# rofuyu/exp-trmf-nips16

Hardware: AMD Instinct MI355X
Metric: als_iterations_per_sec (higher is better)
Workload: dtype f32

## Files before the change

### exp-trmf-nips16_amd/csrc/gram_kernels.hpp

```cpp
#pragma once

#include <type_traits>
#include <utility>

#include "common.hpp"

namespace trmf {

template <typename T> struct Mfma16;
template <> struct Mfma16<float> {
    typedef float acc_t __attribute__((ext_vector_type(4)));
    static __device__ __forceinline__ acc_t mma(float a, float b, acc_t c) {
        return __builtin_amdgcn_mfma_f32_16x16x4f32(a, b, c, 0, 0, 0);
    }
    static __device__ __forceinline__ int row(int lane, int r) { return 4 * (lane >> 4) + r; }
};
template <> struct Mfma16<double> {
    typedef double acc_t __attribute__((ext_vector_type(4)));
    static __device__ __forceinline__ acc_t mma(double a, double b, acc_t c) {
        return __builtin_amdgcn_mfma_f64_16x16x4f64(a, b, c, 0, 0, 0);
    }
    static __device__ __forceinline__ int row(int lane, int r) { return (lane >> 4) + 4 * r; }
};

// ... 486 lines not shown

template <int NT, int KMAX, bool RHS_IN>
__device__ __forceinline__ void quad_factor_solve(quad_f4 (&a4)[NT][KMAX / 4], float (&bz)[NT], float (&x)[NT], int c) {
    constexpr int NR = KMAX / 4;
    float dinv[NT];
#pragma unroll
    for (int q = 0; q < NT; q++) dinv[q] = 0;
    static_for<KMAX>([&](auto J) {
        constexpr int j = decltype(J)::value, qj = j >> 4, cj = j & 15, Rj = j >> 2, ij = j & 3;
        {
            const float inv = __builtin_amdgcn_rsqf(row_bcast<cj>(a4[qj][Rj][ij]));
            float u[NT], nu[NT];
#pragma unroll
            for (int q = qj; q < NT; q++) {
                u[q] = a4[q][Rj][ij] * inv;
                if (q == qj && c <= cj) u[q] = 0;
                a4[q][Rj][ij] = u[q];
                nu[q] = -u[q];
            }
            if constexpr (!RHS_IN) {
                const float zj = row_bcast<cj>(bz[qj]) * inv;
#pragma unroll
                for (int q = qj; q < NT; q++) bz[q] = fmaf(-u[q], zj, bz[q]);
                if (c == cj) bz[qj] = zj;
            }
            if (c == cj) dinv[qj] = inv;
            static_for<NR>([&](auto Rx) {
                constexpr int R = decltype(Rx)::value, qs = (4 * R) >> 4;
                if constexpr (4 * R + 3 > j) {
#pragma unroll
                    for (int q = qs; q < NT; q++) a4[q][R] = __builtin_amdgcn_mfma_f32_4x4x1f32(nu[qs], u[q], a4[q][R], 2, R & 3, 0);
                }
            });
            __builtin_amdgcn_sched_barrier(0);
        }
    });
#pragma unroll
    for (int q = 0; q < NT; q++) x[q] = 0;
    if constexpr (RHS_IN) {
        if (c == 15) x[NT - 1] = -1.0f;
#pragma unroll
        for (int q = 0; q < NT; q++) bz[q] = 0;
    }
    static_for<KMAX>([&](auto Jr) {
        constexpr int j = KMAX - 1 - decltype(Jr)::value, qj = j >> 4, cj = j & 15, Rj = j >> 2, ij = j & 3;
        {
            float part = 0;
#pragma unroll
            for (int q = qj; q < NT; q++) part = fmaf(a4[q][Rj][ij], x[q], part);
            const float sum = row16_allsum_dpp(part);
            const float xv = (bz[qj] - sum) * dinv[qj];
            if (c == cj) x[qj] = xv;
        }
    });
}

struct QuadStream {
    uint32_t pr[5];
    uint32_t step;
    uint32_t long_m1;
    __device__ __forceinline__ uint32_t row_ptr_at(int i) const {
        return i == 0 ? pr[0] : i == 1 ? pr[1] : i == 2 ? pr[2] : i == 3 ? pr[3] : pr[4];
    }
    __device__ __forceinline__ bool skips(int r) const { return row_ptr_at(r + 1) - row_ptr_at(r) - 1u >= long_m1; }
    __device__ __forceinline__ GramDesc first() const {
        GramDesc d{0, 0, -1};
        for (int r = 0; r < 4; r++)
            if (!skips(r)) { d = GramDesc{row_ptr_at(r), row_ptr_at(r + 1), r}; break; }
        return d;
    }
    __device__ __forceinline__ void operator()(GramDesc &d) const {
        if (d.row < 0) return;
        d.e0 += step;
        if (d.e0 < d.end) return;
        int r = d.row + 1;
        while (r < 4 && skips(r)) r++;
        if (r < 4) d = GramDesc{row_ptr_at(r), row_ptr_at(r + 1), r};
        else d = GramDesc{0, 0, -1};
    }
};

constexpr int kQuadWaves = 3;
constexpr int quad_waves(int NT) { return NT >= 4 ? 2 : kQuadWaves; }
constexpr bool quad_row_end(int NT, int KMAX) { return (NT == 3 && KMAX == 40) || (NT == 4 && KMAX == 56); }
#if !defined(TRMF_UNIT_BODIES)
template <int NT, int KMAX>
__global__ void fsolve_quad_kernel(const uint32_t *__restrict__ ptr,
                                                          const uint32_t *__restrict__ idx,
                                                          const float *__restrict__ val,
                                                          const float *__restrict__ X,
                                                          float *__restrict__ F, uint32_t row_begin,
                                                          uint32_t row_end, int k, float lambda,
                                                          uint32_t zero_row, uint32_t long_m1);
template <int NT, int KMAX>
__global__ void fsolve_quad_long_kernel(SplitRows sp, float *__restrict__ F, int k, float lambda);
#else
template <int NT, int KMAX, bool LONG>
__device__ __forceinline__ void fsolve_quad_body(const uint32_t *__restrict__ ptr,
                                                          const uint32_t *__restrict__ idx,
                                                          const float *__restrict__ val,
                                                          const float *__restrict__ X,
                                                          float *__restrict__ F, uint32_t row_begin,
                                                          uint32_t row_end, int k, float lambda,
                                                          uint32_t zero_row, uint32_t long_m1, const SplitRows &sp) {
    static_assert(sizeof(real) == 4, "quad F-solve is the fp32 path");
    constexpr int KP = kTile * NT;
    constexpr int SLAB = quad_slab_floats<NT>();
    __shared__ __attribute__((aligned(16))) float lds_slab[4][SLAB];
    const int wave = threadIdx.x >> 6, lane = threadIdx.x & 63;
    const int grp = lane >> 4, c = lane & 15;
    const uint32_t row0 = LONG ? sp.begin + (blockIdx.x * 4u + (uint32_t)wave) * 4u : row_begin + (blockIdx.x * 4u + (uint32_t)wave) * 4u;
    if (row0 >= (LONG ? sp.end : row_end)) return;
    float *S = lds_slab[wave];
    typedef float f4 __attribute__((ext_vector_type(4)));

    quad_f4 a4[NT][KMAX / 4];
    float bz[NT];
#pragma unroll
    for (int q = 0; q < NT; q++) {
        bz[q] = 0;
#pragma unroll
        for (int s = 0; s < KMAX; s++) a4[q][s >> 2][s & 3] = (s == kTile * q + c) ? 1.0f : 0.0f;
    }
    bool mine = false;

    QuadStream stream;
    stream.step = 4u * kRingDepth;
    stream.long_m1 = long_m1;
    {
        const uint32_t rr = row0 + (uint32_t)(lane < 5 ? lane : 4);
        const uint32_t lim = LONG ? sp.end : row_end;
        const uint32_t v = (LONG ? sp.first : ptr)[rr < lim ? rr : lim];
#pragma unroll
        for (int i = 0; i < 5; i++) stream.pr[i] = (uint32_t)__builtin_amdgcn_readlane((int)v, i);
    }

    GramState<NT> st;
    st.clear();
    constexpr bool PAD = KMAX <= kTile * NT - 8;
    auto finalize = [&](int sys) {
        if constexpr (!PAD) {
#pragma unroll
            for (int q = 0; q < NT; q++) {
                st.b[q] += __shfl_xor(st.b[q], 16, kWave);
                st.b[q] += __shfl_xor(st.b[q], 32, kWave);
            }
        }
        int t = 0;
#pragma unroll
        for (int ti = 0; ti < NT; ti++)
#pragma unroll
            for (int tj = ti; tj < NT; tj++, t++) {
                f4 v = st.acc[t];
                if (ti == tj) {
#pragma unroll
                    for (int r = 0; r < 4; r++)
                        if (c == 4 * grp + r) v[r] += (kTile * ti + c < k) ? lambda : 1.0f;
                }
                *reinterpret_cast<f4 *>(&S[quad_slab_col_offset<NT>(tj) + c * (kTile * (tj + 1) + 4) + kTile * ti + 4 * grp]) = v;
            }
        __builtin_amdgcn_fence(__ATOMIC_ACQ_REL, "wavefront");
        __builtin_amdgcn_wave_barrier();
        if (grp == sys) {
            mine = true;
#pragma unroll
            for (int q = 0; q < NT; q++) {
                if constexpr (!PAD) bz[q] = st.b[q];
#pragma unroll
                for (int s4 = 0; s4 < KMAX / 4; s4++) {
                    if (4 * s4 <= kTile * q + 15)
                        a4[q][s4] = *reinterpret_cast<const f4 *>(&S[quad_slab_col_offset<NT>(q) + c * (kTile * (q + 1) + 4) + 4 * s4]);
                }
            }
        }
        __builtin_amdgcn_fence(__ATOMIC_ACQ_REL, "wavefront");
        __builtin_amdgcn_wave_barrier();
        st.clear();
    };

    if constexpr (LONG) {
        for (int sys = 0; sys < 4; sys++) {
            if (stream.row_ptr_at(sys + 1) == stream.row_ptr_at(sys)) continue;
            load_row_sum<NT, !PAD>(st, sp, stream.row_ptr_at(sys), lane);
            finalize(sys);
        }
    } else {
        float nowq[NT];
#pragma unroll
        for (int q = 0; q < NT; q++) nowq[q] = 0;
        gram_ring<NT, kRingDepth, true, false, PAD, false, quad_row_end(NT, KMAX)>(st, idx, val, X, zero_row, 4u, lane, nowq, stream.first(), stream,
                                                    finalize);
    }

    float x[NT];
    quad_factor_solve<NT, KMAX, PAD>(a4, bz, x, c);
    if (mine) {
        RealVec<NT> o;
#pragma unroll
        for (int q = 0; q < NT; q++) o.v[q] = (kTile * q + c < k) ? x[q] : 0.0f;
        const uint32_t orow = LONG ? sp.rows[row0 + (uint32_t)grp] : row0 + (uint32_t)grp;
        *reinterpret_cast<RealVec<NT> *>(F + (size_t)orow * KP + NT * c) = o;
    }
}
template <int NT, int KMAX>
__global__ __launch_bounds__(256, quad_waves(NT)) void fsolve_quad_kernel(const uint32_t *__restrict__ ptr,
                                                          const uint32_t *__restrict__ idx,
                                                          const float *__restrict__ val,
                                                          const float *__restrict__ X,
                                                          float *__restrict__ F, uint32_t row_begin,
                                                          uint32_t row_end, int k, float lambda,
                                                          uint32_t zero_row, uint32_t long_m1) {
    fsolve_quad_body<NT, KMAX, false>(ptr, idx, val, X, F, row_begin, row_end, k, lambda, zero_row, long_m1, SplitRows{});
}
template <int NT, int KMAX>
__global__ __launch_bounds__(256, quad_waves(NT) - 1) void fsolve_quad_long_kernel(SplitRows sp, float *__restrict__ F, int k, float lambda) {
    fsolve_quad_body<NT, KMAX, true>(nullptr, nullptr, nullptr, nullptr, F, 0u, 0u, k, lambda, 0u, 0u, sp);
}
#endif

#endif

#if !defined(TRMF_UNIT_BODIES)
template <int NT, bool RHS_PAD, bool PACKED>
__global__ void gram_x_kernel(const uint32_t *__restrict__ ptr,
                                                     const uint32_t *__restrict__ idx,
                                                     const real *__restrict__ val,
                                                     const real *__restrict__ Hf,
                                                     real *__restrict__ G, real *__restrict__ Bv,
                                                     uint32_t row_begin, uint32_t row_end, int k,
                                                     uint32_t zero_row, size_t gs, uint32_t long_thresh, const uint32_t *__restrict__ order);
template <int NT, bool RHS_PAD, bool PACKED>
__global__ void gram_x_long_kernel(SplitRows sp, real *__restrict__ G, real *__restrict__ Bv, int k, size_t gs);
template <int NT, bool RHS_PAD>
__global__ void gram_part_kernel(const uint32_t *__restrict__ idx, const real *__restrict__ val, const real *__restrict__ X,
                                 const uint32_t *__restrict__ items, uint32_t item_begin, uint32_t item_end,
                                 real *__restrict__ slab, uint32_t stride, uint32_t zero_row);
#else
template <int NT, bool RHS_PAD>
__global__ __launch_bounds__(256) void gram_part_kernel(const uint32_t *__restrict__ idx, const real *__restrict__ val,
                                                        const real *__restrict__ X, const uint32_t *__restrict__ items,
                                                        uint32_t item_begin, uint32_t item_end, real *__restrict__ slab,
                                                        uint32_t stride, uint32_t zero_row) {
    typedef typename Mfma16<real>::acc_t acc_t;
    constexpr int NTT = NT * (NT + 1) / 2;
    const int wave = threadIdx.x >> 6, lane = threadIdx.x & 63;
    const uint32_t item = item_begin + blockIdx.x * 4u + (uint32_t)wave;
    if (item >= item_end) return;
    const uint32_t p0 = (uint32_t)__builtin_amdgcn_readfirstlane((int)items[2 * item]);
    const uint32_t p1 = (uint32_t)__builtin_amdgcn_readfirstlane((int)items[2 * item + 1]);
    GramState<NT> st;
    st.clear();
    real nowq[NT];
#pragma unroll
    for (int q = 0; q < NT; q++) nowq[q] = 0;
    if (p1 > p0)
        gram_ring<NT, kRingDepth, true, false, RHS_PAD>(st, idx, val, X, zero_row, 4u, lane, nowq, GramDesc{p0, p1, 0},
                                                        SingleRowStream{4u * kRingDepth}, [](int) {});
    real *p = slab + (size_t)item * stride;
#pragma unroll
    for (int t = 0; t < NTT; t++) *reinterpret_cast<acc_t *>(p + t * 4 * kWave + 4 * lane) = st.acc[t];
    if constexpr (!RHS_PAD) {
#pragma unroll
        for (int q = 0; q < NT; q++) p[NTT * 4 * kWave + q * kWave + lane] = st.b[q];
    }
}

template <int NT, bool RHS_PAD, bool PACKED, bool LONG>
__device__ __forceinline__ void gram_x_body(const uint32_t *__restrict__ ptr,
                                                     const uint32_t *__restrict__ idx,
                                                     const real *__restrict__ val,
                                                     const real *__restrict__ Hf,
                                                     real *__restrict__ G, real *__restrict__ Bv,
                                                     uint32_t row_begin, uint32_t row_end, int k,
                                                     uint32_t zero_row, size_t gs, uint32_t long_thresh, const SplitRows &sp,
                                                     const uint32_t *__restrict__ order) {
    constexpr int KP = kTile * NT;
    const int wave = threadIdx.x >> 6, lane = threadIdx.x & 63;
    const int g = lane >> 4, c = lane & 15;
    GramState<NT> st;
    uint32_t row;
    if constexpr (LONG) {
        const uint32_t li = sp.begin + blockIdx.x * 4u + (uint32_t)wave;
        if (li >= sp.end) return;
        row = (uint32_t)__builtin_amdgcn_readfirstlane((int)sp.rows[li]);
        load_row_sum<NT, !RHS_PAD>(st, sp, (uint32_t)__builtin_amdgcn_readfirstlane((int)sp.first[li]), lane);
    } else {
    row = row_begin + blockIdx.x * (blockDim.x >> 6) + (uint32_t)wave;
    if (row >= row_end) return;
    if (order) row = (uint32_t)__builtin_amdgcn_readfirstlane((int)order[row]);
    const uint32_t p0 = (uint32_t)__builtin_amdgcn_readfirstlane((int)ptr[row]);
    const uint32_t p1 = (uint32_t)__builtin_amdgcn_readfirstlane((int)ptr[row + 1]);
    if (p1 - p0 >= long_thresh) return;

    st.clear();
    real nowq[NT];
#pragma unroll
    for (int q = 0; q < NT; q++) nowq[q] = 0;
    if (p1 > p0)
        gram_ring<NT, kRingDepth, true, false, RHS_PAD>(st, idx, val, Hf, zero_row, 4u, lane, nowq, GramDesc{p0, p1, 0},
// ... 108 lines not shown
```

### exp-trmf-nips16_amd/csrc/kernel_units.hpp

```cpp
#pragma once

#if defined(TRMF_UNIT) || defined(TRMF_SINGLE_UNIT)
#define TRMF_UNIT_BODIES 1
#endif
#if !defined(TRMF_UNIT) || TRMF_UNIT == 1
#include "gram_kernels.hpp"
#endif
#if !defined(TRMF_UNIT) || TRMF_UNIT == 2
#include "cg_kernels.hpp"
#endif
#if defined(TRMF_UNIT) && TRMF_UNIT == 4
#include "cg_kernels.hpp"
#include "gram_kernels.hpp"
#include "full_kernels.hpp"
#endif
#if !defined(TRMF_UNIT) || TRMF_UNIT == 5
#include "heldout_kernels.hpp"
#endif
#if !defined(TRMF_UNIT) || TRMF_UNIT == 6
#include "forecast_kernels.hpp"
#endif
#if !defined(TRMF_UNIT) || TRMF_UNIT == 7
#include "online_kernels.hpp"
#endif
#if !defined(TRMF_UNIT) || TRMF_UNIT == 8
#include "uncertainty_kernels.hpp"
#endif
#if !defined(TRMF_UNIT)
#include "cg_persist_args.hpp"
#elif TRMF_UNIT == 3
#include "cg_persist.hpp"
#endif
#if defined(TRMF_SINGLE_UNIT)
#include "cg_persist.hpp"
#endif

namespace trmf {

#define TRMF_HV_SIG (XParams, XState *, HvVecs, TileShard, int, int, const uint32_t *, const real *, const real *, const double *, double *, const PeerTable *, int, int)
#define TRMF_HV_KQS(X, MODE, SHARD, NTH)                           \
    X void hv_tile_kernel<MODE, 8, SHARD, NTH> TRMF_HV_SIG;        \
    X void hv_tile_kernel<MODE, 16, SHARD, NTH> TRMF_HV_SIG;       \
    X void hv_tile_kernel<MODE, 24, SHARD, NTH> TRMF_HV_SIG;       \
    X void hv_tile_kernel<MODE, 32, SHARD, NTH> TRMF_HV_SIG;       \
    X void hv_tile_kernel<MODE, 40, SHARD, NTH> TRMF_HV_SIG;       \
    X void hv_tile_kernel<MODE, 48, SHARD, NTH> TRMF_HV_SIG;       \
    X void hv_tile_kernel<MODE, 56, SHARD, NTH> TRMF_HV_SIG;       \
    X void hv_tile_kernel<MODE, 64, SHARD, NTH> TRMF_HV_SIG;
#define TRMF_UNIT_HV(X, SHARD, NTH)                                                                                   \
    TRMF_HV_KQS(X, HV_GRAD, SHARD, NTH) TRMF_HV_KQS(X, HV_CG_FIRST, SHARD, NTH) TRMF_HV_KQS(X, HV_CG_STEP, SHARD, NTH) TRMF_HV_KQS(X, HV_PLAIN, SHARD, NTH)

#define TRMF_PERSIST_SIG (XParams, XState *, PersistArgs)
#define TRMF_PERSIST_KQS(X, SHARD, NTH)                                  \
    X void cg_persist_kernel<8, SHARD, NTH> TRMF_PERSIST_SIG;            \
    X void cg_persist_kernel<16, SHARD, NTH> TRMF_PERSIST_SIG;           \
    X void cg_persist_kernel<24, SHARD, NTH> TRMF_PERSIST_SIG;           \
    X void cg_persist_kernel<32, SHARD, NTH> TRMF_PERSIST_SIG;           \
    X void cg_persist_kernel<40, SHARD, NTH> TRMF_PERSIST_SIG;           \
    X void cg_persist_kernel<48, SHARD, NTH> TRMF_PERSIST_SIG;           \
    X void cg_persist_kernel<56, SHARD, NTH> TRMF_PERSIST_SIG;           \
    X void cg_persist_kernel<64, SHARD, NTH> TRMF_PERSIST_SIG;
#define TRMF_UNIT_PERSIST(X) TRMF_PERSIST_KQS(X, false, 256) TRMF_PERSIST_KQS(X, true, 256) TRMF_PERSIST_KQS(X, false, 512)

#define TRMF_FSOLVE_SIG (const uint32_t *, const uint32_t *, const real *, const real *, real *, uint32_t, uint32_t, int, real, uint32_t, uint32_t)
#define TRMF_FSOLVE_LONG_SIG (SplitRows, real *, int, real)
#if defined(TRMF_F32)
#define TRMF_FSOLVE_ONE(X, NT, KMAX) X void fsolve_quad_kernel<NT, KMAX> TRMF_FSOLVE_SIG;
#define TRMF_FSOLVE_LONG_ONE(X, NT, KMAX) X void fsolve_quad_long_kernel<NT, KMAX> TRMF_FSOLVE_LONG_SIG;
#else
#define TRMF_FSOLVE_ONE(X, NT, KMAX) X void fsolve_mfma_kernel<NT, KMAX> TRMF_FSOLVE_SIG;
#define TRMF_FSOLVE_LONG_ONE(X, NT, KMAX) X void fsolve_mfma_long_kernel<NT, KMAX> TRMF_FSOLVE_LONG_SIG;
#endif
#define TRMF_GRAMX_SIG (const uint32_t *, const uint32_t *, const real *, const real *, real *, real *, uint32_t, uint32_t, int, uint32_t, size_t, uint32_t, const uint32_t *)
#define TRMF_GRAMX_LONG_SIG (SplitRows, real *, real *, int, size_t)
#define TRMF_GRAM_PART_SIG (const uint32_t *, const real *, const real *, const uint32_t *, uint32_t, uint32_t, real *, uint32_t, uint32_t)
#define TRMF_SPLIT_NT(X, NT)                                               \
    X void gram_part_kernel<NT, true> TRMF_GRAM_PART_SIG;                  \
    X void gram_part_kernel<NT, false> TRMF_GRAM_PART_SIG;                 \
    X void gram_x_long_kernel<NT, true, true> TRMF_GRAMX_LONG_SIG;         \
    X void gram_x_long_kernel<NT, true, false> TRMF_GRAMX_LONG_SIG;        \
    X void gram_x_long_kernel<NT, false, true> TRMF_GRAMX_LONG_SIG;        \
    X void gram_x_long_kernel<NT, false, false> TRMF_GRAMX_LONG_SIG;
#define TRMF_UNIT_SPLIT(X)                                                                                                   \
    TRMF_FSOLVE_LONG_ONE(X, 1, 8) TRMF_FSOLVE_LONG_ONE(X, 1, 16) TRMF_FSOLVE_LONG_ONE(X, 2, 24) TRMF_FSOLVE_LONG_ONE(X, 2, 32) \
    TRMF_FSOLVE_LONG_ONE(X, 3, 40) TRMF_FSOLVE_LONG_ONE(X, 3, 48) TRMF_FSOLVE_LONG_ONE(X, 4, 56) TRMF_FSOLVE_LONG_ONE(X, 4, 64) \
    TRMF_SPLIT_NT(X, 1) TRMF_SPLIT_NT(X, 2) TRMF_SPLIT_NT(X, 3) TRMF_SPLIT_NT(X, 4)
#define TRMF_GRAMX_NT(X, NT)                                     \
    X void gram_x_kernel<NT, true, true> TRMF_GRAMX_SIG;         \
    X void gram_x_kernel<NT, true, false> TRMF_GRAMX_SIG;        \
    X void gram_x_kernel<NT, false, true> TRMF_GRAMX_SIG;        \
    X void gram_x_kernel<NT, false, false> TRMF_GRAMX_SIG;
#define TRMF_LOSS_SIG (const uint32_t *, const uint32_t *, const real *, const real *, const real *, double *, uint32_t, uint32_t, uint32_t)
#define TRMF_UNIT_GRAM(X)                                                                                                    \
    TRMF_FSOLVE_ONE(X, 1, 8) TRMF_FSOLVE_ONE(X, 1, 16) TRMF_FSOLVE_ONE(X, 2, 24) TRMF_FSOLVE_ONE(X, 2, 32)                   \
    TRMF_FSOLVE_ONE(X, 3, 40) TRMF_FSOLVE_ONE(X, 3, 48) TRMF_FSOLVE_ONE(X, 4, 56) TRMF_FSOLVE_ONE(X, 4, 64)                  \
    TRMF_GRAMX_NT(X, 1) TRMF_GRAMX_NT(X, 2) TRMF_GRAMX_NT(X, 3) TRMF_GRAMX_NT(X, 4)                                         \
    X void loss_kernel<1> TRMF_LOSS_SIG; X void loss_kernel<2> TRMF_LOSS_SIG; X void loss_kernel<3> TRMF_LOSS_SIG; X void loss_kernel<4> TRMF_LOSS_SIG;

#define TRMF_APPLY_SHARED_SIG (XParams, const XState *, int, const real *, const real *, const real *, const real *, const real *, int, real *, int, double *, int, int, int)
#define TRMF_FULL_NT(X, NT)                                                                                                              \
    X void spmm_rows_kernel<NT>(const uint32_t *, const uint32_t *, const real *, const real *, real *, uint32_t, uint32_t, uint32_t, uint32_t);  \
    X void spmm_part_kernel<NT>(const uint32_t *, const real *, const real *, const uint32_t *, uint32_t, uint32_t, real *, uint32_t);  \
    X void dense_tn_mfma_kernel<NT>(const real *, int, int, const real *, double *);                                                    \
    X void small_gram_mfma_kernel<NT>(const real *, int, int, double *);                                                                \
    X void chol_wave_kernel<NT>(const real *, real *, int);                                                                             \
    X void apply_shared_mfma_kernel<NT> TRMF_APPLY_SHARED_SIG;
#define TRMF_UNIT_FULL(X) TRMF_FULL_NT(X, 1) TRMF_FULL_NT(X, 2) TRMF_FULL_NT(X, 3) TRMF_FULL_NT(X, 4)

#define TRMF_UNIT_HELDOUT(X)                                                                                                 \
    X void heldout_eval_kernel<0>(HeldoutArgs); X void heldout_eval_kernel<1>(HeldoutArgs); X void heldout_eval_kernel<2>(HeldoutArgs); \
    X void heldout_eval_kernel<3>(HeldoutArgs); X void heldout_eval_kernel<4>(HeldoutArgs);

#define TRMF_UNIT_FORECAST(X)                                                                                                \
    X void forecast_score_kernel<0>(ScoreArgs); X void forecast_score_kernel<1>(ScoreArgs); X void forecast_score_kernel<2>(ScoreArgs); \
    X void forecast_score_kernel<3>(ScoreArgs); X void forecast_score_kernel<4>(ScoreArgs);

#define TRMF_UNIT_ONLINE(X)                                                                                                  \
    X void assim_factor_kernel<1>(AssimFactorArgs); X void assim_factor_kernel<2>(AssimFactorArgs);                          \
    X void assim_factor_kernel<3>(AssimFactorArgs); X void assim_factor_kernel<4>(AssimFactorArgs);

#define TRMF_UNIT_UNCERTAINTY(X)                                                                                             \
    X void noise_resid_kernel<0>(NoiseResidArgs); X void noise_resid_kernel<1>(NoiseResidArgs); X void noise_resid_kernel<2>(NoiseResidArgs); \
    X void noise_resid_kernel<3>(NoiseResidArgs); X void noise_resid_kernel<4>(NoiseResidArgs);                              \
    X void forecast_dist_kernel<0>(DistArgs); X void forecast_dist_kernel<1>(DistArgs); X void forecast_dist_kernel<2>(DistArgs); \
    X void forecast_dist_kernel<3>(DistArgs); X void forecast_dist_kernel<4>(DistArgs);

#define TRMF_DEFINE_KERNEL template __global__

}
```

### exp-trmf-nips16_amd/csrc/session.hpp

```cpp
#pragma once

#include "session_xphase.hpp"

extern "C" char **environ;

namespace trmf {

struct TrmfSessionImpl : SessionXPhase {
    ~TrmfSessionImpl() {
        if (stream) (void)hipStreamSynchronize(stream);
        if (side) (void)hipStreamSynchronize(side);
        if (aux_theta) (void)hipStreamSynchronize(aux_theta);
        for (auto &e : events) {
            hipEvent_t all[] = {e.f0, e.fk0, e.fk1, e.f1, e.xg1, e.x1, e.lv1};
            for (hipEvent_t ev : all) if (ev) (void)hipEventDestroy(ev);
        }
        for (hipEvent_t ev : {gx0, gx1, gx2, fs0, fs1, fs2, ts0, ts1}) if (ev) (void)hipEventDestroy(ev);
        release_p2p();
        for (hipEvent_t ev : {ov_b, ov_c[0], ov_c[1], ov_c[2], ov_c[3], emu_ready, emu_end}) if (ev) (void)hipEventDestroy(ev);
        if (side) (void)hipStreamDestroy(side);
        for (hipEvent_t ev : {theta_fork, theta_done}) if (ev) (void)hipEventDestroy(ev);
        if (cg_note) (void)hipHostFree(cg_note);
        StreamCache::release(aux_theta);
        StreamCache::release(stream);
// ... 600 lines not shown
            }
            TRMF_EVREC(ev.x1, stream);
            if (doL) {
                if (verbose) {
                    log_norm(theta.p, (size_t)nlag * k, &L->normLV);
                    fprintf(stderr, ">> iter %d LV(%d %d) %g\n", iter1, nlag, k, host_double(&L->normLV));
                }
                const bool under_f = nlag > 0 && it + 1 < iters && overlap_ok();
                if (under_f) {
                    if (join_theta()) return kFail;
                    TRMF_HIP_CHECK(hipEventRecord(theta_fork, stream));
                    TRMF_HIP_CHECK(hipStreamWaitEvent(aux_theta, theta_fork, 0));
                    if (theta_solve(aux_theta)) return kFail;
                    TRMF_EVREC(ev.lv1, aux_theta);
                    TRMF_HIP_CHECK(hipEventRecord(theta_done, aux_theta));
                    theta_pending = true;
                    continue;
                }
                if (join_theta() || theta_solve(stream)) return kFail;
                if (log_norms || verbose) log_norm(theta.p, (size_t)nlag * k, &L->normLV);
                if (verbose) fprintf(stderr, ">> iter %d LV %g\n", iter1, host_double(&L->normLV));
            }
            TRMF_EVREC(ev.lv1, stream);
        }
        return join_theta();
    }
    int take_snapshot() {
        const size_t nw = (size_t)(T + 1) * KP, nh = (size_t)(n + 1) * KP, nt = (size_t)nlag * k;
        FillStreamScope fill(stream);
        if (snapW.alloc(nw, false) || snapH.alloc(nh, false) || snapT.alloc(nt, false)) return kFail;
        TRMF_HIP_CHECK(hipMemcpyAsync(snapW.p, W.p, nw * sizeof(real), hipMemcpyDeviceToDevice, stream));
        TRMF_HIP_CHECK(hipMemcpyAsync(snapH.p, H.p, nh * sizeof(real), hipMemcpyDeviceToDevice, stream));
        if (nt) TRMF_HIP_CHECK(hipMemcpyAsync(snapT.p, theta.p, nt * sizeof(real), hipMemcpyDeviceToDevice, stream));
        snap_iter = iter;
        return 0;
    }
    int mark() {
        if (sync()) return kFail;
        const size_t nw = (size_t)(T + 1) * KP, nh = (size_t)(n + 1) * KP, nt = (size_t)nlag * k;
        FillStreamScope fill(stream);
        if (markW.alloc(nw, false) || markH.alloc(nh, false) || markT.alloc(nt, false)) return kFail;
        TRMF_HIP_CHECK(hipMemcpyAsync(markW.p, W.p, nw * sizeof(real), hipMemcpyDeviceToDevice, stream));
        TRMF_HIP_CHECK(hipMemcpyAsync(markH.p, H.p, nh * sizeof(real), hipMemcpyDeviceToDevice, stream));
        if (nt) TRMF_HIP_CHECK(hipMemcpyAsync(markT.p, theta.p, nt * sizeof(real), hipMemcpyDeviceToDevice, stream));
        TRMF_HIP_CHECK(hipStreamSynchronize(stream));
        mark_iter = iter;
        return 0;
    }
    int rewind() {
        if (mark_iter < 0) { set_error("rewind: no mark has been set"); return kFail; }
        const size_t nw = (size_t)(T + 1) * KP, nh = (size_t)(n + 1) * KP, nt = (size_t)nlag * k;
        if (markW.n != nw || markH.n != nh) { set_error("rewind: the session has grown since the mark (append_rows)"); return kFail; }
        if (sync()) return kFail;
        TRMF_HIP_CHECK(hipMemcpyAsync(W.p, markW.p, nw * sizeof(real), hipMemcpyDeviceToDevice, stream));
        TRMF_HIP_CHECK(hipMemcpyAsync(H.p, markH.p, nh * sizeof(real), hipMemcpyDeviceToDevice, stream));
        if (nt) TRMF_HIP_CHECK(hipMemcpyAsync(theta.p, markT.p, nt * sizeof(real), hipMemcpyDeviceToDevice, stream));
        iter = mark_iter;
        if (snap_iter >= 0 && take_snapshot()) return kFail;
        TRMF_HIP_CHECK(hipStreamSynchronize(stream));
        return 0;
    }
    int persist_recover(const XState &hx) {
        if (snap_iter < 0) { set_error("persistent CG kernel timed out and no snapshot exists"); return kFail; }
        const int redo = iter - snap_iter;
        if (verbose || getenv("TRMF_P2P_VERBOSE"))
            fprintf(stderr, ">> persistent CG kernel: a poll ran into its bound (exchange %lld, tile %lld, %s missing; is another process using the GPU?): "
                    "repeating %d iteration(s) with one launch per CG step\n", hx.p2p_diag[0], hx.p2p_diag[1], hx.p2p_diag[2] == 1 ? "records" : "halo rows", redo);
        persist_state = -1; persist_failed = true;
        persist_note = "the persistent kernel ran into a poll bound after iteration " + std::to_string(snap_iter) + ": one launch per CG step since";
        const size_t nw = (size_t)(T + 1) * KP, nh = (size_t)(n + 1) * KP, nt = (size_t)nlag * k;
        TRMF_HIP_CHECK(hipMemsetAsync(&xstate.p->p2p_error, 0, sizeof(int), stream));
        TRMF_HIP_CHECK(hipMemcpyAsync(W.p, snapW.p, nw * sizeof(real), hipMemcpyDeviceToDevice, stream));
        TRMF_HIP_CHECK(hipMemcpyAsync(H.p, snapH.p, nh * sizeof(real), hipMemcpyDeviceToDevice, stream));
        if (nt) TRMF_HIP_CHECK(hipMemcpyAsync(theta.p, snapT.p, nt * sizeof(real), hipMemcpyDeviceToDevice, stream));
        iter = snap_iter;
        if (run(redo)) return kFail;
        TRMF_HIP_CHECK(hipStreamSynchronize(stream));
        snapW.release(); snapH.release(); snapT.release(); snap_iter = -1;
        return 0;
    }

    int sync(bool recover = true) {
        TRMF_HIP_CHECK(hipStreamSynchronize(stream));
#if defined(TRMF_PERSIST_PROF)
        if (persist_prof.p) {
            std::vector<long long> hp((size_t)2 * kProfIters * kProfSlots + 2 * (size_t)kPersistMaxTiles);
            TRMF_HIP_CHECK(hipMemcpy(hp.data(), persist_prof.p, hp.size() * sizeof(long long), hipMemcpyDeviceToHost));
            for (int sel = 0; sel < 2; sel++) {
                const long long t0 = hp[(size_t)sel * kProfIters * kProfSlots];
                for (int i = 0; i < kProfIters; i++) {
                    const long long *r = hp.data() + ((size_t)sel * kProfIters + i) * kProfSlots;
                    if (!r[0] && !r[3]) continue;
                    fprintf(stderr, "PERSIST_PROF tile %s row %2d:", sel ? "mid" : "0  ", i);
                    for (int q = 0; q < kProfSlots; q++) fprintf(stderr, " %8.2f", r[q] ? (r[q] - t0) * 0.01 : 0.0);
                    fprintf(stderr, "  us\n");
                }
            }
            {
                const long long *q = hp.data() + (size_t)2 * kProfIters * kProfSlots;
                long long base = 0;
                for (int t = 0; t < nbt; t++) if (q[2 * t] && (!base || q[2 * t] < base)) base = q[2 * t];
                fprintf(stderr, "PERSIST_TILES");
                for (int t = 0; t < nbt; t++) fprintf(stderr, " %.2f/%.2f", (q[2 * t] - base) * 0.01, (q[2 * t + 1] - base) * 0.01);
                fprintf(stderr, "\n");
            }
        }
#endif
        if (persist_state == 1 && comm->world == 1) {
            XState hx;
            TRMF_HIP_CHECK(hipMemcpy(&hx, xstate.p, sizeof hx, hipMemcpyDeviceToHost));
            if (hx.p2p_error && recover) return persist_recover(hx);
            if (hx.p2p_error) { set_error("persistent CG kernel: an exchange between workgroups timed out"); return kFail; }
            if (recover && snap_iter >= 0 && snap_iter != iter && take_snapshot()) return kFail;
        } else if (persist_state == 1 || (persist_shard_state == 1 && x_form == kXTsPersist)) {
            XState hx;
            TRMF_HIP_CHECK(hipMemcpy(&hx, xstate.p, sizeof hx, hipMemcpyDeviceToHost));
            if (hx.p2p_error) { set_error("persistent CG kernel: an exchange between workgroups timed out (is another process using the GPU? TRMF_PERSIST=0 selects the launch-per-step path)"); return kFail; }
        }
        if (p2p.on) {
            XState hx;
            TRMF_HIP_CHECK(hipMemcpy(&hx, xstate.p, sizeof hx, hipMemcpyDeviceToHost));
            if (hx.p2p_error) {
                char msg[256];
                snprintf(msg, sizeof msg, "time-sharded CG: a peer-to-peer exchange timed out (TRMF_CG=p2p): rank %d, message %lld, launch %lld, "
                         "peer %lld: expected epoch %lld, flag %lld", comm->rank, hx.p2p_diag[0] / 1000000, hx.p2p_diag[0] / 1000 % 1000 - 1,
                         hx.p2p_diag[0] % 1000, hx.p2p_diag[1], hx.p2p_diag[2]);
                set_error(msg);
                if (test_env("TRMF_P2P_DEBUG")) {
                    std::vector<double> hp((size_t)P_NSLOTS * xp.pstride);
                    TRMF_HIP_CHECK(hipMemcpy(hp.data(), pbase(), hp.size() * sizeof(double), hipMemcpyDeviceToHost));
                    fprintf(stderr, "[p2p debug] rank %d: %s\n  stop_it %d cg_iter %d rho %.17g %.17g %.17g gnorm %.17g cgtol %.9g\n", comm->rank, msg,
                            hx.stop_it, hx.cg_iter, hx.rho_hist[0], hx.rho_hist[1], hx.rho_hist[2], hx.gnorm, (double)hx.cgtol);
                    for (int a = 0; a < P_NSLOTS; a++) {
                        double t = 0; int nz = 0;
                        for (int q = 0; q < xp.pstride; q++) { t += hp[(size_t)a * xp.pstride + q]; nz += hp[(size_t)a * xp.pstride + q] != 0; }
                        fprintf(stderr, "  partial array %2d: sum %.17g (%d nonzero)\n", a, t, nz);
                    }
                }
                return kFail;
            }
        }
        return 0;
    }

    int stats(TrmfIterStats *out, int cap) {
        if (sync()) return kFail;
        const int avail = std::min(iter, std::min(kLogCap, kEventRing));
        const int cnt = std::min(cap, avail);
        for (int q = 0; q < cnt; q++) {
            const int it0 = iter - cnt + q;
            DeviceIterLog hl;
            TRMF_HIP_CHECK(hipMemcpy(&hl, log.p + (it0 % kLogCap), sizeof hl, hipMemcpyDeviceToHost));
            PhaseEvents &ev = events[it0 % kEventRing];
            TrmfIterStats &o = out[q];
            o.normF = hl.normF; o.normX = hl.normX; o.normLV = hl.normLV;
            o.f = hl.x.f; o.fnew = hl.x.fnew; o.actred = hl.x.actred; o.prered = hl.x.prered;
            o.gnorm = hl.x.gnorm; o.cg_rnorm = hl.x.cg_rnorm; o.cg_iter = hl.x.cg_iter; o.accepted = hl.x.accepted; o.delta = hl.x.delta;
            o.cg_rnorm_direct = hl.x.rho_direct >= 0 ? std::sqrt(hl.x.rho_direct) : -1.0;
            o.ms_F = o.ms_X = o.ms_LV = o.ms_F_kernel = o.ms_X_gram = -1;
            if (ev_valid.size() != (size_t)kEventRing || !ev_valid[it0 % kEventRing]) continue;
            (void)hipEventElapsedTime(&o.ms_X_gram, ev.f1, ev.xg1);
            (void)hipEventElapsedTime(&o.ms_F, ev.f0, ev.f1);
            (void)hipEventElapsedTime(&o.ms_F_kernel, ev.fk0, ev.fk1);
            (void)hipEventElapsedTime(&o.ms_X, ev.f1, ev.x1);
            (void)hipEventElapsedTime(&o.ms_LV, ev.x1, ev.lv1);
        }
// ... 415 lines not shown
```

### exp-trmf-nips16_amd/csrc/session_fphase.hpp

```cpp
#pragma once

#include "session_transport.hpp"

namespace trmf {

struct SessionFPhase : SessionTransport {
    template <int NT_, bool PAD_> void launch_gram_part(const LongRows &L, uint32_t lo, uint32_t hi, const uint32_t *idx, const real *val,
                                                        const real *X, uint32_t zero_row) {
        const uint32_t i0 = L.first[lo], i1 = L.first[hi];
        if (i1 <= i0) return;
        hipLaunchKernelGGL((gram_part_kernel<NT_, PAD_>), dim3((i1 - i0 + 3) / 4), dim3(256), 0, stream, idx, val, X, L.d_items.p, i0, i1,
                           part_slab.p, part_stride, zero_row);
        if (i1 - i0 > hi - lo) {
            const uint32_t bpr = (uint32_t)((part_stride * sizeof(real) / 16 + 255) / 256);
            hipLaunchKernelGGL(split_reduce_kernel, dim3(bpr * (hi - lo)), dim3(256), 0, stream, L.d_first.p, part_slab.p, part_stride, lo, hi, bpr);
        }
    }
    template <int NT_, int KMAX_> int launch_fsolve_mfma(uint32_t rb, uint32_t re) {
        const uint32_t rows = re - rb;
        if (rows == 0) return 0;
#if !defined(TRMF_F32)
        if (longF.any()) {
            uint32_t lo, hi;
            longF.range(rb, re, lo, hi);
            if (hi > lo) {
                launch_gram_part<NT_, false>(longF, lo, hi, Yc_idx.p, Yc_val.p, W.p, (uint32_t)T);
                hipLaunchKernelGGL((fsolve_mfma_long_kernel<NT_, KMAX_>), dim3((hi - lo + 3) / 4), dim3(256), 0, stream, split_view(longF, lo, hi), H.p, k, (real)lambdaI);
            }
        }
        hipLaunchKernelGGL((fsolve_mfma_kernel<NT_, KMAX_>), dim3((rows + 3) / 4), dim3(256), 0, stream,
                           Yc_ptr.p, Yc_idx.p, Yc_val.p, W.p, H.p, rb, re, k, (real)lambdaI, (uint32_t)T, longF.thresh - 1u);
#endif
        return 0;
    }
    template <int NT_, int KMAX_> int launch_fsolve_quad(uint32_t rb, uint32_t re) {
        const uint32_t rows = re - rb;
        if (rows == 0) return 0;
#if defined(TRMF_F32)
        if (longF.any()) {
            uint32_t lo, hi;
            longF.range(rb, re, lo, hi);
            if (hi > lo) {
                launch_gram_part<NT_, (KMAX_ <= kTile * NT_ - 8)>(longF, lo, hi, Yc_idx.p, Yc_val.p, W.p, (uint32_t)T);
                hipLaunchKernelGGL((fsolve_quad_long_kernel<NT_, KMAX_>), dim3((hi - lo + 15) / 16), dim3(256), 0, stream, split_view(longF, lo, hi), H.p, k, (real)lambdaI);
            }
        }
        if (longF.any()) { uint32_t lo, hi; longF.range(rb, re, lo, hi); if (hi - lo == rows) return 0; }
        const dim3 grid((rows + 15) / 16), block(256);
        hipLaunchKernelGGL((fsolve_quad_kernel<NT_, KMAX_>), grid, block, 0, stream, Yc_ptr.p,
                           Yc_idx.p, Yc_val.p, W.p, H.p, rb, re, k, (real)lambdaI, (uint32_t)T, longF.thresh - 1u);
#endif
        return 0;
    }
    int launch_fsolve_rows(uint32_t rb, uint32_t re) {
        if (generic) {
            if (re > rb)
                hipLaunchKernelGGL(gram_generic_kernel<true>, dim3(std::min<uint32_t>(kGenBlocks, re - rb)), dim3(256), gram_generic_lds(k), stream,
                                   Yc_ptr.p, Yc_idx.p, Yc_val.p, W.p, rb, re, k, KP, NT, (real)lambdaI, gen_scratch.p, (size_t)0, H.p);
            return 0;
        }
        return with_kq(KMAX, [&](auto KM) {
            constexpr int KMAX_ = decltype(KM)::value, NT_ = (KMAX_ + kTile - 1) / kTile;
            if (sizeof(real) == 4) launch_fsolve_quad<NT_, KMAX_>(rb, re);
            else launch_fsolve_mfma<NT_, KMAX_>(rb, re);
        }) ? 0 : unsupported_rank();
    }
    int overlap_chunks() {
        if (comm->world <= 1 || full || host_col_ptr.empty()) return 0;
        if (const char *e = test_env("TRMF_FOVERLAP")) { const int c = atoi(e); return c <= 0 ? 0 : std::max(2, std::min(kMaxChunks, c)); }
        uint64_t rows = 0;
        for (int r = 0; r < comm->world; r++) rows = std::max<uint64_t>(rows, fbounds[r + 1] - fbounds[r]);
        uint64_t thresh = kOverlapBytes;
        if (const char *e = test_env("TRMF_FOVERLAP_BYTES")) thresh = std::max<uint64_t>(1, strtoull(e, nullptr, 10));
        const uint64_t bytes = rows * KP * sizeof(real);
        return bytes >= thresh ? (int)std::max<uint64_t>(2, std::min<uint64_t>(kMaxChunks, bytes / thresh)) : 0;
    }
    int fsolve(PhaseEvents &ev) {
        if (fs_mode == kShardMeasure && fs_calls == 2) {
            const int m = decide_shard(fs0, fs1, fs2, "F-solve");
            if (m < 0) return kFail;
            fs_mode = m;
        }
        const bool replicate = fs_mode == kShardOff, measure = fs_mode == kShardMeasure && fs_calls == 1;
        const uint32_t rb = replicate ? 0u : (uint32_t)fbounds[comm->rank];
        const uint32_t re = replicate ? (uint32_t)n : (uint32_t)fbounds[comm->rank + 1];
        const int C = fs_mode == kShardOn ? overlap_chunks() : 0;
        if (C >= 2) {
            const int W_ = comm->world;
            if (!side) {
                TRMF_HIP_CHECK(hipStreamCreateWithFlags(&side, hipStreamNonBlocking));
                TRMF_HIP_CHECK(hipEventCreateWithFlags(&ov_b, hipEventDisableTiming));
                for (hipEvent_t &e : ov_c) TRMF_HIP_CHECK(hipEventCreateWithFlags(&e, hipEventDisableTiming));
            }
            if (fchunks != C || fcut.size() != (size_t)W_ * (C + 1)) {
                fchunks = C; fcut.resize((size_t)W_ * (C + 1));
                for (int r = 0; r < W_; r++) {
                    const uint64_t n0 = host_col_ptr[fbounds[r]], n1 = host_col_ptr[fbounds[r + 1]];
                    fcut[(size_t)r * (C + 1)] = fbounds[r]; fcut[(size_t)r * (C + 1) + C] = fbounds[r + 1];
                    for (int c = 1; c < C; c++)
                        fcut[(size_t)r * (C + 1) + c] = (uint64_t)(std::lower_bound(host_col_ptr.begin() + fbounds[r], host_col_ptr.begin() + fbounds[r + 1],
                                                                                   n0 + (n1 - n0) * c / C) - host_col_ptr.begin());
                }
            }
            const uint64_t rowbytes = (uint64_t)KP * sizeof(real);
            const uint64_t *mine = fcut.data() + (size_t)comm->rank * (C + 1);
            TRMF_EVREC(ev.fk0, stream);
            for (int c = 0; c < C; c++) {
                if (launch_fsolve_rows((uint32_t)mine[c], (uint32_t)mine[c + 1])) return kFail;
                if (c + 1 < C) TRMF_HIP_CHECK(hipEventRecord(ov_c[c], stream));
            }
            TRMF_EVREC(ev.fk1, stream);
            TRMF_HIP_CHECK(hipGetLastError());
            fs_calls++;
            std::vector<uint64_t> gb(W_), ge(W_);
            for (int c = 0; c < C; c++) {
                for (int r = 0; r < W_; r++) { gb[r] = fcut[(size_t)r * (C + 1) + c] * rowbytes; ge[r] = fcut[(size_t)r * (C + 1) + c + 1] * rowbytes; }
                if (c + 1 < C) {
                    TRMF_HIP_CHECK(hipStreamWaitEvent(side, ov_c[c], 0));
                    if (comm->allgatherv_ranges(H.p, gb.data(), ge.data(), side)) return kFail;
                } else {
                    TRMF_HIP_CHECK(hipEventRecord(ov_b, side));
                    if (comm->allgatherv_ranges(H.p, gb.data(), ge.data(), stream)) return kFail;
                    TRMF_HIP_CHECK(hipStreamWaitEvent(stream, ov_b, 0));
                }
            }
            return 0;
        }
        if (measure) TRMF_HIP_CHECK(hipEventRecord(fs0, stream));
        TRMF_EVREC(ev.fk0, stream);
        if (launch_fsolve_rows(rb, re)) return kFail;
        TRMF_EVREC(ev.fk1, stream);
        TRMF_HIP_CHECK(hipGetLastError());
        fs_calls++;
        if (replicate) return 0;
        if (measure) TRMF_HIP_CHECK(hipEventRecord(fs1, stream));
        if (gather_rows(H.p, fbounds, (size_t)KP * sizeof(real))) return kFail;
// ... 105 lines not shown
```

Baseline: 1245.

## Launch F-solve quad kernel with one wave per block and add timing stamps

```diff
diff --git a/exp-trmf-nips16_amd/csrc/gram_kernels.hpp b/exp-trmf-nips16_amd/csrc/gram_kernels.hpp
--- a/exp-trmf-nips16_amd/csrc/gram_kernels.hpp
+++ b/exp-trmf-nips16_amd/csrc/gram_kernels.hpp
@@ -592,7 +592,33 @@
 
 constexpr int kQuadWaves = 3;
 constexpr int quad_waves(int NT) { return NT >= 4 ? 2 : kQuadWaves; }
+constexpr int kQuadBlockWaves = 1;
 constexpr bool quad_row_end(int NT, int KMAX) { return (NT == 3 && KMAX == 40) || (NT == 4 && KMAX == 56); }
+#if defined(TRMF_FSOLVE_STAMPS)
+#define TRMF_STAMPS_PARAM , unsigned long long *stamps
+#define TRMF_STAMPS_ARG stamps
+constexpr int kStampWords = 8;
+#define TRMF_STAMP(i)                                                                                                         \
+    do {                                                                                                                      \
+        if constexpr (!LONG) {                                                                                                \
+            __builtin_amdgcn_sched_barrier(0);                                                                                \
+            const unsigned long long rt_ = __builtin_amdgcn_s_memrealtime(), ck_ = __builtin_amdgcn_s_memtime();              \
+            if (lane == 0) {                                                                                                  \
+                unsigned long long *o_ = stamps + (size_t)gw * kStampWords;                                                   \
+                o_[2 * (i)] = rt_; o_[2 * (i) + 1] = ck_;                                                                     \
+                if ((i) == 0) {                                                                                               \
+                    o_[6] = (unsigned long long)__builtin_amdgcn_s_getreg((31 << 11) | 4) | ((unsigned long long)__builtin_amdgcn_s_getreg((31 << 11) | 20) << 32); \
+                    o_[7] = row0;                                                                                             \
+                }                                                                                                             \
+            }                                                                                                                 \
+            __builtin_amdgcn_sched_barrier(0);                                                                                \
+        }                                                                                                                     \
+    } while (0)
+#else
+#define TRMF_STAMPS_PARAM
+#define TRMF_STAMPS_ARG nullptr
+#define TRMF_STAMP(i) do { } while (0)
+#endif
 #if !defined(TRMF_UNIT_BODIES)
 template <int NT, int KMAX>
 __global__ void fsolve_quad_kernel(const uint32_t *__restrict__ ptr,
@@ -601,7 +627,7 @@
                                                           const float *__restrict__ X,
                                                           float *__restrict__ F, uint32_t row_begin,
                                                           uint32_t row_end, int k, float lambda,
-                                                          uint32_t zero_row, uint32_t long_m1);
+                                                          uint32_t zero_row, uint32_t long_m1 TRMF_STAMPS_PARAM);
 template <int NT, int KMAX>
 __global__ void fsolve_quad_long_kernel(SplitRows sp, float *__restrict__ F, int k, float lambda);
 #else
@@ -612,15 +638,19 @@
                                                           const float *__restrict__ X,
                                                           float *__restrict__ F, uint32_t row_begin,
                                                           uint32_t row_end, int k, float lambda,
-                                                          uint32_t zero_row, uint32_t long_m1, const SplitRows &sp) {
+                                                          uint32_t zero_row, uint32_t long_m1, const SplitRows &sp,
+                                                          unsigned long long *stamps) {
     static_assert(sizeof(real) == 4, "quad F-solve is the fp32 path");
     constexpr int KP = kTile * NT;
     constexpr int SLAB = quad_slab_floats<NT>();
-    __shared__ __attribute__((aligned(16))) float lds_slab[4][SLAB];
-    const int wave = threadIdx.x >> 6, lane = threadIdx.x & 63;
+    constexpr int WPB = LONG ? 4 : kQuadBlockWaves;
+    __shared__ __attribute__((aligned(16))) float lds_slab[WPB][SLAB];
+    const int wave = WPB == 1 ? 0 : threadIdx.x >> 6, lane = threadIdx.x & 63;
     const int grp = lane >> 4, c = lane & 15;
-    const uint32_t row0 = LONG ? sp.begin + (blockIdx.x * 4u + (uint32_t)wave) * 4u : row_begin + (blockIdx.x * 4u + (uint32_t)wave) * 4u;
+    const uint32_t gw = blockIdx.x * (uint32_t)WPB + (uint32_t)wave;
+    const uint32_t row0 = (LONG ? sp.begin : row_begin) + gw * 4u;
     if (row0 >= (LONG ? sp.end : row_end)) return;
+    TRMF_STAMP(0);
     float *S = lds_slab[wave];
     typedef float f4 __attribute__((ext_vector_type(4)));
 
@@ -701,9 +731,11 @@
         gram_ring<NT, kRingDepth, true, false, PAD, false, quad_row_end(NT, KMAX)>(st, idx, val, X, zero_row, 4u, lane, nowq, stream.first(), stream,
                                                     finalize);
     }
+    TRMF_STAMP(1);
 
     float x[NT];
     quad_factor_solve<NT, KMAX, PAD>(a4, bz, x, c);
+    TRMF_STAMP(2);
     if (mine) {
         RealVec<NT> o;
 #pragma unroll
@@ -713,18 +745,18 @@
     }
 }
 template <int NT, int KMAX>
-__global__ __launch_bounds__(256, quad_waves(NT)) void fsolve_quad_kernel(const uint32_t *__restrict__ ptr,
+__global__ __launch_bounds__(64 * kQuadBlockWaves, quad_waves(NT)) void fsolve_quad_kernel(const uint32_t *__restrict__ ptr,
                                                           const uint32_t *__restrict__ idx,
                                                           const float *__restrict__ val,
                                                           const float *__restrict__ X,
                                                           float *__restrict__ F, uint32_t row_begin,
                                                           uint32_t row_end, int k, float lambda,
-                                                          uint32_t zero_row, uint32_t long_m1) {
-    fsolve_quad_body<NT, KMAX, false>(ptr, idx, val, X, F, row_begin, row_end, k, lambda, zero_row, long_m1, SplitRows{});
+                                                          uint32_t zero_row, uint32_t long_m1 TRMF_STAMPS_PARAM) {
+    fsolve_quad_body<NT, KMAX, false>(ptr, idx, val, X, F, row_begin, row_end, k, lambda, zero_row, long_m1, SplitRows{}, TRMF_STAMPS_ARG);
 }
 template <int NT, int KMAX>
 __global__ __launch_bounds__(256, quad_waves(NT) - 1) void fsolve_quad_long_kernel(SplitRows sp, float *__restrict__ F, int k, float lambda) {
-    fsolve_quad_body<NT, KMAX, true>(nullptr, nullptr, nullptr, nullptr, F, 0u, 0u, k, lambda, 0u, 0u, sp);
+    fsolve_quad_body<NT, KMAX, true>(nullptr, nullptr, nullptr, nullptr, F, 0u, 0u, k, lambda, 0u, 0u, sp, nullptr);
 }
 #endif
 
diff --git a/exp-trmf-nips16_amd/csrc/kernel_units.hpp b/exp-trmf-nips16_amd/csrc/kernel_units.hpp
--- a/exp-trmf-nips16_amd/csrc/kernel_units.hpp
+++ b/exp-trmf-nips16_amd/csrc/kernel_units.hpp
@@ -65,7 +65,12 @@
 #define TRMF_FSOLVE_SIG (const uint32_t *, const uint32_t *, const real *, const real *, real *, uint32_t, uint32_t, int, real, uint32_t, uint32_t)
 #define TRMF_FSOLVE_LONG_SIG (SplitRows, real *, int, real)
 #if defined(TRMF_F32)
-#define TRMF_FSOLVE_ONE(X, NT, KMAX) X void fsolve_quad_kernel<NT, KMAX> TRMF_FSOLVE_SIG;
+#if defined(TRMF_FSOLVE_STAMPS)
+#define TRMF_FSOLVE_QUAD_SIG (const uint32_t *, const uint32_t *, const real *, const real *, real *, uint32_t, uint32_t, int, real, uint32_t, uint32_t, unsigned long long *)
+#else
+#define TRMF_FSOLVE_QUAD_SIG TRMF_FSOLVE_SIG
+#endif
+#define TRMF_FSOLVE_ONE(X, NT, KMAX) X void fsolve_quad_kernel<NT, KMAX> TRMF_FSOLVE_QUAD_SIG;
 #define TRMF_FSOLVE_LONG_ONE(X, NT, KMAX) X void fsolve_quad_long_kernel<NT, KMAX> TRMF_FSOLVE_LONG_SIG;
 #else
 #define TRMF_FSOLVE_ONE(X, NT, KMAX) X void fsolve_mfma_kernel<NT, KMAX> TRMF_FSOLVE_SIG;
diff --git a/exp-trmf-nips16_amd/csrc/session.hpp b/exp-trmf-nips16_amd/csrc/session.hpp
--- a/exp-trmf-nips16_amd/csrc/session.hpp
+++ b/exp-trmf-nips16_amd/csrc/session.hpp
@@ -706,6 +706,13 @@
 
     int sync(bool recover = true) {
         TRMF_HIP_CHECK(hipStreamSynchronize(stream));
+#if defined(TRMF_FSOLVE_STAMPS)
+        if (const char *path = getenv("TRMF_FSOLVE_STAMPS"); path && fsolve_stamps.p) {
+            std::vector<unsigned long long> hs(fsolve_stamps.n);
+            TRMF_HIP_CHECK(hipMemcpy(hs.data(), fsolve_stamps.p, hs.size() * sizeof(unsigned long long), hipMemcpyDeviceToHost));
+            if (FILE *f = fopen(path, "wb")) { fwrite(hs.data(), sizeof(unsigned long long), hs.size(), f); fclose(f); }
+        }
+#endif
 #if defined(TRMF_PERSIST_PROF)
         if (persist_prof.p) {
             std::vector<long long> hp((size_t)2 * kProfIters * kProfSlots + 2 * (size_t)kPersistMaxTiles);
diff --git a/exp-trmf-nips16_amd/csrc/session_fphase.hpp b/exp-trmf-nips16_amd/csrc/session_fphase.hpp
--- a/exp-trmf-nips16_amd/csrc/session_fphase.hpp
+++ b/exp-trmf-nips16_amd/csrc/session_fphase.hpp
@@ -46,12 +46,22 @@
             }
         }
         if (longF.any()) { uint32_t lo, hi; longF.range(rb, re, lo, hi); if (hi - lo == rows) return 0; }
-        const dim3 grid((rows + 15) / 16), block(256);
+        const uint32_t quads = (rows + 3) / 4;
+        const dim3 grid((quads + kQuadBlockWaves - 1) / kQuadBlockWaves), block(64 * kQuadBlockWaves);
+#if defined(TRMF_FSOLVE_STAMPS)
+        if (fsolve_stamps.n != (size_t)grid.x * kQuadBlockWaves * kStampWords && fsolve_stamps.alloc((size_t)grid.x * kQuadBlockWaves * kStampWords)) return kFail;
+        hipLaunchKernelGGL((fsolve_quad_kernel<NT_, KMAX_>), grid, block, 0, stream, Yc_ptr.p,
+                           Yc_idx.p, Yc_val.p, W.p, H.p, rb, re, k, (real)lambdaI, (uint32_t)T, longF.thresh - 1u, fsolve_stamps.p);
+#else
         hipLaunchKernelGGL((fsolve_quad_kernel<NT_, KMAX_>), grid, block, 0, stream, Yc_ptr.p,
                            Yc_idx.p, Yc_val.p, W.p, H.p, rb, re, k, (real)lambdaI, (uint32_t)T, longF.thresh - 1u);
 #endif
-        return 0;
-    }
+#endif
+        return 0;
+    }
+#if defined(TRMF_FSOLVE_STAMPS)
+    DevBuf<unsigned long long> fsolve_stamps;
+#endif
     int launch_fsolve_rows(uint32_t rb, uint32_t re) {
         if (generic) {
             if (re > rb)
```

Result: no change. 1251, median of 6 (+0.6%).
